# huzaifakhan04/truely-real-time-ai-generated-video-detection-framework-for-social-platforms

Measured on AMD Instinct MI355X. Metric: frames/sec (detect+embed+drift) 720p, higher is better.
Workload: dtype f32

## Files before the change

### truely-real-time-ai-generated-video-detection-framework-for-social-platforms_amd/csrc/trl_api.hip

```cpp
#include <stdarg.h>
#include <stdio.h>
#include <string.h>
#include <stdlib.h>

#include "trl_ctx.h"

static thread_local char g_err[512] = "";
int g_trl_no_fnconv = 0;
int g_trl_pnet_gate = 0;

#include <mutex>
namespace {
std::mutex g_gate_mu;
hipEvent_t g_gate_ev[64] = {};
bool g_gate_set[64] = {};
}
int trl_gate_wait(trl_ctx* c, hipStream_t s) {
    const int d = c->cfg.device;
    if (!g_trl_pnet_gate || d < 0 || d >= 64) return TRL_OK;
    std::lock_guard<std::mutex> lk(g_gate_mu);
    if (g_gate_set[d]) TRL_HIP(hipStreamWaitEvent(s, g_gate_ev[d], 0));
    return TRL_OK;
}
int trl_gate_record(trl_ctx* c, hipStream_t s) {
// ... 694 lines not shown
    TRL_HIP(hipSetDevice(c->cfg.device));
    const int capF = nb;
    Arena& A = c->arena;
    TRL_CHECK(trl_ensure(c, A, (size_t)capF * 32 + (1u << 20)));
    A.reset();
    CascadeBufs& B = c->cb;
    B = CascadeBufs();
    B.n = 1; B.H = H; B.W = W;
    B.cbox = (int32_t*)A.alloc((size_t)capF * 32);
    int32_t* total = (int32_t*)A.alloc(64);
    std::vector<int32_t> hb((size_t)nb * 8, 0);
    for (int i = 0; i < nb; i++) {
        const float* b = h_boxes + 4 * i;
        const int bx = (int)truncf(b[0]), by = (int)truncf(b[1]), bex = (int)truncf(b[2]), bey = (int)truncf(b[3]);
        const int x = bx < 1 ? 1 : bx, y = by < 1 ? 1 : by, ex = bex > W ? W : bex, ey = bey > H ? H : bey;
        hb[8 * i + 1] = y - 1; hb[8 * i + 2] = x - 1; hb[8 * i + 3] = ey - (y - 1); hb[8 * i + 4] = ex - (x - 1);
    }
    TRL_HIP(hipMemcpyAsync(B.cbox, hb.data(), hb.size() * 4, hipMemcpyHostToDevice, s));
    TRL_HIP(hipMemcpyAsync(total, &nb, 4, hipMemcpyHostToDevice, s));
    TRL_HIP(hipStreamSynchronize(s));
    c->scratch.reset();
    TRL_CHECK(trl_ensure(c, c->scratch, (size_t)nb * 700 * 1024 + (4u << 20)));
    if (net == 24) {
        float* pool1 = (float*)c->scratch.alloc((size_t)nb * 11 * 11 * 28 * 4);
        TRL_CHECK(trl_launch_rnet_front(c, d_frame, H, W, total, 0, nb, pool1, s));
        TRL_CHECK(trl_run_rnet_tail(c, pool1, nb, d_out, s, total, 0));
    } else {
        float* pool1 = (float*)c->scratch.alloc((size_t)nb * 23 * 23 * 32 * 4);
        TRL_CHECK(trl_launch_onet_front(c, d_frame, H, W, total, 0, nb, pool1, s));
        TRL_CHECK(trl_run_onet_tail(c, pool1, nb, d_out, s, total, 0));
    }
    TRL_HIP(hipStreamSynchronize(s));
    B = CascadeBufs();
    return TRL_OK;
}

int trl_debug_onet(trl_ctx* c, const float* d_crops, int n, float* d_out, void* stream) {
    if (!c || !c->have_weights || !d_crops || !d_out || n <= 0) { trl_set_error("bad argument"); return TRL_ERR_INVALID; }
    TRL_CHECK(check_idle(c));
    c->scratch.reset();
    TRL_CHECK(trl_ensure(c, c->scratch, (size_t)n * 640 * 1024 + (4u << 20)));
    return trl_run_onet(c, d_crops, n, d_out, (hipStream_t)stream);
}
int trl_debug_crop_resize(trl_ctx* c, const uint8_t* d_frames, int n, int H, int W, const int32_t* d_rect, const uint8_t* d_valid,
                          float* d_faces, void* stream) {
    if (!c || !d_frames || !d_rect || !d_valid || !d_faces || n <= 0) { trl_set_error("bad argument"); return TRL_ERR_INVALID; }
    return trl_launch_crop_resize80(d_frames, n, H, W, d_rect, d_valid, d_faces, (hipStream_t)stream);
}
int trl_debug_crop_aligned(trl_ctx* c, const uint8_t* d_frames, int n, int H, int W, const float* d_pts, const uint8_t* d_valid, int S,
                           int rgb, float* d_faces, void* stream) {
    if (!c || !d_frames || !d_pts || !d_valid || !d_faces || n <= 0 || H < 1 || W < 1 || S < 1) { trl_set_error("bad argument"); return TRL_ERR_INVALID; }
    return trl_launch_crop_aligned(d_frames, n, H, W, d_pts, d_valid, S, rgb != 0, d_faces, (hipStream_t)stream);
}
int trl_debug_nms_tiers(trl_ctx* c, int small_tier, int full_tier) {
    TRL_CHECK(check_idle(c));
    if ((small_tier && (small_tier < 16 || small_tier > 3072 || (small_tier & 3))) || (full_tier && (full_tier < 16 || full_tier > 3072 || (full_tier & 3)))) {
        trl_set_error("tiers must be multiples of 4 in [16, 3072]");
        return TRL_ERR_INVALID;
    }
    if (small_tier) c->nms_small = small_tier;
    if (full_tier) c->nms_full = full_tier;
    return TRL_OK;
}
int trl_debug_list_stats(trl_ctx* c, long long* h_out8) {
    if (!c || !h_out8) { trl_set_error("null argument"); return TRL_ERR_INVALID; }
    const int32_t* f = c->h_pinned + 4;
    unsigned long long used = 0;
    memcpy(&used, f + 8, 8);
    int mx = 0;
    for (int l = 0; l < 32; l++) if (f[16 + l] > mx) mx = f[16 + l];
    h_out8[0] = c->last_attempts; h_out8[1] = f[10]; h_out8[2] = (long long)used; h_out8[3] = (long long)c->cb.spill_cap;
    h_out8[4] = c->cb.capF; h_out8[5] = c->cb.lay.S; h_out8[6] = mx; h_out8[7] = f[6];
    return TRL_OK;
}

int trl_debug_option(trl_ctx* c, const char* key, int value) {
    if (!key) { trl_set_error("null key"); return TRL_ERR_INVALID; }
    if (!strcmp(key, "no_fnconv")) { g_trl_no_fnconv = value ? 1 : 0; return TRL_OK; }
    if (!strcmp(key, "pnet_gate")) { g_trl_pnet_gate = value ? 1 : 0; return TRL_OK; }
    TRL_CHECK(check_idle(c));
    if (!strcmp(key, "rnet_chunk") && value >= 16) { c->rnet_chunk = value; return TRL_OK; }
    if (!strcmp(key, "onet_chunk") && value >= 16) { c->onet_chunk = value; return TRL_OK; }
    if (!strcmp(key, "pnet_screen") && (value == 0 || value == 1)) { c->pnet_screen = value; return TRL_OK; }
    trl_set_error("unknown option '%s' (or value %d out of range)", key, value);
    return TRL_ERR_INVALID;
}

int trl_debug_pnet_screen_bound(trl_ctx* c, float* A, float* B, int* on) {
    if (!c || !A || !B || !on) { trl_set_error("null argument"); return TRL_ERR_INVALID; }
    *A = c->pnet_scrA; *B = c->pnet_scrB; *on = c->pnet_screen_ok && c->pnet_screen;
    return TRL_OK;
}

int trl_debug_batch_capacity(trl_ctx* c, float t2_per_frame, float t3_per_frame, int* last_attempts) {
    if (!c) { trl_set_error("null context"); return TRL_ERR_INVALID; }
    if (t2_per_frame > 0.f) c->t2_per_frame = t2_per_frame;
    if (t3_per_frame > 0.f) c->t3_per_frame = t3_per_frame;
    if (last_attempts) *last_attempts = c->last_attempts;
    return TRL_OK;
}

int trl_debug_stage_totals(trl_ctx* c, int32_t* h_out2) {
    if (!c || !h_out2) { trl_set_error("null argument"); return TRL_ERR_INVALID; }
    h_out2[0] = c->h_pinned[4 + 4]; h_out2[1] = c->h_pinned[4 + 5];
    return TRL_OK;
}

int trl_debug_pnet_run(trl_ctx* c, int run) {
    if (!c || run < 0 || run > 64) { trl_set_error("bad argument"); return TRL_ERR_INVALID; }
    c->pnet_run = run;
    return TRL_OK;
}

int trl_debug_pnet_span(trl_ctx* c, int reset, double* ms_sum, int32_t* launches) {
    if (!c || !ms_sum || !launches) { trl_set_error("null argument"); return TRL_ERR_INVALID; }
    *ms_sum = 0.0; *launches = 0;
    if (!c->pnet_clk) return TRL_OK;
    TRL_CHECK(check_idle(c));
    TRL_HIP(hipSetDevice(c->cfg.device));
    TRL_HIP(hipDeviceSynchronize());
    unsigned long long t[2] = {0, 0};
    int khz = 0;
    TRL_HIP(hipMemcpy(t, c->pnet_clk + 36, sizeof t, hipMemcpyDeviceToHost));
    TRL_HIP(hipDeviceGetAttribute(&khz, hipDeviceAttributeWallClockRate, c->cfg.device));
    if (khz > 0) *ms_sum = (double)t[0] / (double)khz;
    *launches = (int32_t)t[1];
    if (reset) TRL_HIP(hipMemset(c->pnet_clk + 36, 0, 16));
    return TRL_OK;
}

int trl_debug_pnet_kernel_ms(trl_ctx* c, float* ms) {
    if (!c || !ms) { trl_set_error("null argument"); return TRL_ERR_INVALID; }
    *ms = c->pnet_kernel_ms;
    return TRL_OK;
}

int trl_debug_timings(trl_ctx* c, float* out4) {
    if (!c || !out4) return TRL_ERR_INVALID;
    out4[0] = c->last_ms[0]; out4[1] = c->last_ms[1]; out4[2] = c->last_ms[2]; out4[3] = c->last_ms[3];
    return TRL_OK;
}

}
```

### truely-real-time-ai-generated-video-detection-framework-for-social-platforms_amd/csrc/trl_cascade.hip

```cpp
#include "trl_ctx.h"
#include <stdlib.h>
#include <string.h>


namespace {

__device__ __forceinline__ uint32_t f2ord(float f) {
    uint32_t u = __float_as_uint(f);
    return (u & 0x80000000u) ? ~u : (u | 0x80000000u);
}

__device__ void block_bitonic(uint64_t* key, uint32_t* id, int P) {
    for (int k = 2; k <= P; k <<= 1) {
        for (int j = k >> 1; j > 0; j >>= 1) {
            for (int t = threadIdx.x; t < P; t += blockDim.x) {
                const int u = t ^ j;
                if (u > t) {
                    const bool up = ((t & k) == 0);
                    const uint64_t a = key[t], b = key[u];
                    if ((a > b) == up) {
                        key[t] = b; key[u] = a;
                        const uint32_t ia = id[t]; id[t] = id[u]; id[u] = ia;
                    }
                }
// ... 1022 lines not shown
    size_t spill = c->spill_hint;
    {
        size_t per_frame = 0;
        for (int l = 0; l < L; l++) if (G.capl[l] > lds_full) per_frame += spill_need(G.capl[l], W, H);
        if (capF > lds_full) per_frame += 3 * spill_need(capF, W, H);
        size_t up_front = per_frame * (size_t)n;
        if (up_front > (8ull << 30)) up_front = 8ull << 30;
        if (up_front > spill) spill = up_front;
    }
    Arena& A = c->arena;
    Arena& X = c->scratch;
    if (resume) {
        A.off = B.arena_mark;
        TRL_HIP(hipMemsetAsync(B.flags + FLG_T3, 0, 4, s));
        TRL_HIP(hipMemsetAsync(B.flags + FLG_T3N, 0, 4, s));
        if (resume == 2) { TRL_HIP(hipMemsetAsync(B.flags + FLG_T2, 0, 4, s)); TRL_HIP(hipMemsetAsync(B.flags + FLG_T2N, 0, 4, s)); }
    }
    const size_t need = (size_t)n * ((size_t)G.S * (sizeof(Cand) + 4) + (size_t)L * 8) + (size_t)n * capF * (5 * 3 + 10 + 8) * 4 +
                        (size_t)n * 1024 + spill + (1u << 20);
    if (!resume) {
    TRL_CHECK(trl_ensure(c, A, need));
    A.reset();
    B.lvl_cnt = (int32_t*)A.alloc((size_t)n * L * 4);
    B.lvl_keep_cnt = (int32_t*)A.alloc((size_t)n * L * 4);
    B.lvl_rec = (Cand*)A.alloc((size_t)n * G.S * sizeof(Cand));
    B.lvl_keep_idx = (int32_t*)A.alloc((size_t)n * G.S * 4);
    B.n1 = (int32_t*)A.alloc((size_t)n * 4); B.n2 = (int32_t*)A.alloc((size_t)n * 4); B.n3 = (int32_t*)A.alloc((size_t)n * 4);
    B.s1_box = (float*)A.alloc((size_t)n * capF * 20); B.s2_box = (float*)A.alloc((size_t)n * capF * 20);
    B.s3_box = (float*)A.alloc((size_t)n * capF * 20); B.s3_pts = (float*)A.alloc((size_t)n * capF * 40);
    B.off2 = (int32_t*)A.alloc((size_t)(n + 1) * 4); B.off3 = (int32_t*)A.alloc((size_t)(n + 1) * 4);
    B.cbox = (int32_t*)A.alloc((size_t)n * capF * 32);
    B.flags = (int32_t*)A.alloc(TRL_NFLAGS * 4);
    B.spill = spill ? (char*)A.alloc(spill) : nullptr;
    B.spill_cap = B.spill ? spill : 0;
    if (!B.flags || (spill && !B.spill)) { trl_set_error("cascade workspace allocation failed"); return TRL_ERR_STATE; }
    B.arena_mark = A.off;
    TRL_HIP(hipMemsetAsync(B.flags, 0, TRL_NFLAGS * 4, s));
    }
    const Spill sp{B.spill, (unsigned long long)B.spill_cap, B.flags};
    if (L == 0) {
        TRL_HIP(hipMemsetAsync(B.n1, 0, (size_t)n * 4, s));
        TRL_HIP(hipMemsetAsync(B.n2, 0, (size_t)n * 4, s));
        TRL_HIP(hipMemsetAsync(B.n3, 0, (size_t)n * 4, s));
        TRL_HIP(hipMemsetAsync(B.off2, 0, (size_t)(n + 1) * 4, s));
        TRL_HIP(hipMemsetAsync(B.off3, 0, (size_t)(n + 1) * 4, s));
        if (c->scratch_after_cascade) TRL_CHECK(trl_ensure(c, X, c->scratch_after_cascade));
        return TRL_OK;
    }
    if (!resume) TRL_HIP(hipMemsetAsync(B.lvl_cnt, 0, (size_t)n * L * 4, s));

    if (!resume) c->pnet_ev_used = 0;
    X.reset();
    int chunk[32];
    const bool fused = c->cfg.pnet_mode == 0 && L <= 16;
    if (!fused) {
        size_t mx = 0;
        for (int l = 0; l < L; l++) {
            const LevelGeom& g = c->lv[l];
            const size_t per = trl_pnet_generic_bytes(1, g.h, g.w) + (size_t)g.h * g.w * 12 + (size_t)g.oh * g.ow * 24 + 4096;
            int ch = (int)((size_t)(2048ull << 20) / per);
            if (ch < 1) ch = 1;
            if (ch > n) ch = n;
            chunk[l] = ch;
            if (per * ch > mx) mx = per * ch;
        }
        TRL_CHECK(trl_ensure(c, X, mx + (4u << 20)));
    }
    auto next_ev = [&](std::pair<hipEvent_t, hipEvent_t>*& out) -> int {
        if ((int)c->pnet_ev.size() <= c->pnet_ev_used) {
            hipEvent_t e0, e1;
            TRL_HIP(hipEventCreate(&e0)); TRL_HIP(hipEventCreate(&e1));
            c->pnet_ev.push_back({e0, e1});
        }
        out = &c->pnet_ev[c->pnet_ev_used++];
        return TRL_OK;
    };
    {
        long long c2 = (long long)(c->t2_per_frame * n) + 64, c3 = (long long)(c->t3_per_frame * n) + 64;
        const long long lim = (long long)n * capF;
        c->cap_t2 = (int)(c2 < lim ? c2 : lim);
        c->cap_t3 = (int)(c3 < lim ? c3 : lim);
        const int TRL_CH2 = c->rnet_chunk, TRL_CH3 = c->onet_chunk;
        const int ch2 = c->cap_t2 < TRL_CH2 ? c->cap_t2 : TRL_CH2, ch3 = c->cap_t3 < TRL_CH3 ? c->cap_t3 : TRL_CH3;
        size_t need_x = (size_t)c->cap_t2 * 24 + (size_t)ch2 * (40 * 1024) + (1u << 20);
        const size_t need3 = (size_t)c->cap_t3 * 64 + (size_t)ch3 * (240 * 1024) + (1u << 20);
        if (need3 > need_x) need_x = need3;
        if (fused) { const size_t p = trl_pnet_fused_bytes(c, n, H, W) + (1u << 20); if (p > need_x) need_x = p; }
        if (c->scratch_after_cascade > need_x) need_x = c->scratch_after_cascade;
        TRL_CHECK(trl_ensure(c, X, need_x));
    }
    if (resume) {
    } else if (fused) {
        std::pair<hipEvent_t, hipEvent_t>*pa, *pb;
        c->pnet_ev.reserve(64);
        TRL_CHECK(next_ev(pa)); TRL_CHECK(next_ev(pb));
        hipEvent_t ev[4] = {pa->first, pa->second, pb->first, pb->second};
        TRL_CHECK(trl_pnet_fused_all(c, d_frames, n, H, W, ev, s));
    } else {
        for (int l = 0; l < L; l++) {
            const LevelGeom& g = c->lv[l];
            if (g.oh < 1 || g.ow < 1) continue;
            std::pair<hipEvent_t, hipEvent_t>* pe;
            TRL_CHECK(next_ev(pe));
            TRL_HIP(hipEventRecord(pe->first, s));
            for (int f0 = 0; f0 < n; f0 += chunk[l]) {
                const int nf = (n - f0 < chunk[l]) ? n - f0 : chunk[l];
                X.reset();
                float* lvl = (float*)X.alloc((size_t)nf * g.h * g.w * 12);
                float* heads = (float*)X.alloc((size_t)nf * g.oh * g.ow * 24);
                if (!lvl || !heads) { trl_set_error("pnet generic workspace"); return TRL_ERR_STATE; }
                TRL_CHECK(trl_launch_area_level(d_frames + (size_t)f0 * H * W * 3, nf, H, W, g.h, g.w, lvl, s));
                TRL_CHECK(trl_run_pnet_generic(c, lvl, nf, g.h, g.w, heads, s));
                const size_t total = (size_t)nf * g.oh * g.ow;
                size_t blocks = (total + 255) / 256;
                if (blocks > 16384) blocks = 16384;
                k_pnet_collect<<<(unsigned)blocks, 256, 0, s>>>(heads, nf, f0, g.oh, g.ow, (float)g.scale, c->cfg.thr0, L, l, G.capl[l],
                                                                 G.rec0[l], G.S, B.lvl_cnt, B.lvl_rec, B.flags);
                TRL_LAUNCH_CHECK();
            }
            TRL_HIP(hipEventRecord(pe->second, s));
        }
    }
    int max_capl = 4;
    for (int l = 0; l < L; l++) if (G.capl[l] > max_capl) max_capl = G.capl[l];
    const int full_l = max_capl < lds_full ? max_capl : lds_full, full_f = capF < lds_full ? capF : lds_full;
    const int th_l = max_capl > lds_full ? 1024 : 256, th_f = capF > lds_full ? 1024 : 256;
    const size_t sm_l = Smem::bytes(full_l, th_l), sm_f = Smem::bytes(full_f, th_f);
    TRL_CHECK(set_dyn_smem(k_nms_level, sm_l));
    TRL_CHECK(set_dyn_smem(k_nms_frame, sm_f));
    TRL_CHECK(set_dyn_smem(k_stage2_post, sm_f));
    TRL_CHECK(set_dyn_smem(k_stage3_post, sm_f));
    if (!resume) {
        const int small_cap = full_l < lds_small ? full_l : lds_small;
        const size_t sm_s = Smem::bytes(small_cap);
        k_nms_level<<<n * L, 256, sm_s, s>>>(G, small_cap, 0, small_cap == max_capl ? 1 : 0, W, H, B.lvl_cnt, B.lvl_rec, B.lvl_keep_cnt, B.lvl_keep_idx, B.flags, sp);
        TRL_LAUNCH_CHECK();
        if (small_cap < max_capl) {
            k_nms_level<<<n * L, th_l, sm_l, s>>>(G, full_l, small_cap + 1, 1, W, H, B.lvl_cnt, B.lvl_rec, B.lvl_keep_cnt, B.lvl_keep_idx, B.flags, sp);
            TRL_LAUNCH_CHECK();
        }
    }
    if (!resume) {
        k_nms_frame<<<n, th_f, sm_f, s>>>(G, full_f, capF, W, H, B.lvl_rec, B.lvl_keep_cnt, B.lvl_keep_idx, B.n1, B.s1_box, B.flags, sp);
        TRL_LAUNCH_CHECK();
    }

    const int cap2 = c->cap_t2, cap3 = c->cap_t3;
    if (resume < 3) {
    k_scan_counts<<<1, 256, 0, s>>>(B.n1, n, B.off2, cap2, B.flags, 0);
    TRL_LAUNCH_CHECK();
    k_build_map<<<n, 64, 0, s>>>(B.n1, B.off2, B.s1_box, capF, W, H, B.cbox);
    TRL_LAUNCH_CHECK();
    X.reset();
    float* out6 = (float*)X.alloc((size_t)cap2 * 24);
    {
        const int CH = c->rnet_chunk;
        const size_t mk = X.off;
        for (int t0 = 0; t0 < cap2; t0 += CH) {
            const int nc = (cap2 - t0 < CH) ? cap2 - t0 : CH;
            X.off = mk;
            float* pool1 = (float*)X.alloc((size_t)nc * 11 * 11 * 28 * 4);
            if (!pool1 || !out6) { trl_set_error("rnet workspace"); return TRL_ERR_STATE; }
            TRL_CHECK(trl_launch_rnet_front(c, d_frames, H, W, B.off2 + n, t0, nc, pool1, s));
            TRL_CHECK(trl_run_rnet_tail(c, pool1, nc, out6 + (size_t)t0 * 6, s, B.off2 + n, t0));
        }
    }
    k_stage2_post<<<n, th_f, sm_f, s>>>(full_f, capF, cap2, W, H, c->cfg.thr1, B.n1, B.s1_box, B.off2, out6, B.n2, B.s2_box, sp);
// ... 85 lines not shown
```

### truely-real-time-ai-generated-video-detection-framework-for-social-platforms_amd/csrc/trl_ctx.h

```cpp
#pragma once
#include "trl_common.h"

struct Cand {
    float x1, y1, x2, y2, score;
    float r0, r1, r2, r3;
    int cell;
};

struct LevelGeom {
    double scale;
    int h, w;
    int oh, ow;
};

struct LvLayout {
    int L = 0, S = 0;
    int capl[32] = {0}, rec0[32] = {0};
};
struct CascadeBufs {
    int n = 0, L = 0, H = 0, W = 0;
    LvLayout lay;
    int capF = 0;
    int32_t* lvl_cnt = nullptr;
    Cand* lvl_rec = nullptr;
    int32_t* lvl_keep_cnt = nullptr;
    int32_t* lvl_keep_idx = nullptr;
    int32_t* n1 = nullptr; float* s1_box = nullptr;
    int32_t* n2 = nullptr; float* s2_box = nullptr;
    int32_t* n3 = nullptr; float* s3_box = nullptr;
    float* s3_pts = nullptr;
    int32_t* off2 = nullptr; int32_t* off3 = nullptr;
    int32_t* cbox = nullptr;
    int32_t* flags = nullptr;
    size_t arena_mark = 0;
    char* spill = nullptr;
    size_t spill_cap = 0;
};
enum { TRL_NFLAGS = 64 };

struct trl_ctx {
    trl_config cfg;
    bool have_weights = false;
    char* wdev = nullptr;
    size_t wbytes = 0;
    std::unordered_map<std::string, DevW> W;
    std::unordered_map<std::string, DevV> V;
    Arena arena;
    Arena scratch;
    Arena sims_tmp;
    int32_t* h_pinned = nullptr;
    CascadeBufs cb;
    LevelGeom lv[32];
    hipEvent_t ev_call0 = nullptr, ev_call1 = nullptr;
    std::vector<std::pair<hipEvent_t, hipEvent_t>> pnet_ev;
    int pnet_ev_used = 0;
    float last_ms[4] = {0, 0, 0, 0};
    int pnet_mono1 = 0;
    int pnet_unit = 0;
    float pnet_scrA = 0.f, pnet_scrB = 0.f;
    int pnet_screen_ok = 0;
    int pnet_screen = 1;
    int pnet_run = 0;
    int32_t* pnet_cursor = nullptr;
    unsigned long long* pnet_clk = nullptr;
    bool pnet_prof = false;
    float pnet_kernel_ms = 0.f;
    int dbg_poison = -1;
    float t2_per_frame = 160.f, t3_per_frame = 48.f;
    int cap_t2 = 0, cap_t3 = 0;
    float lvl_hint[32] = {0}, frame_hint = 0.f;
    size_t spill_hint = 0;
    int rnet_chunk = 49152, onet_chunk = 16384;
    int nms_small = 512, nms_full = 2048;
    int last_attempts = 0;
    int resume_stage = 0;
    size_t scratch_after_cascade = 0;
    int rnet_front_mode = -1, onet_front_mode = -1;
    struct Pending {
        bool active = false; int attempt = 0;
        const uint8_t* frames = nullptr; int n = 0, H = 0, W = 0;
        float* box = nullptr; float* prob = nullptr; int32_t* rect = nullptr; uint8_t* valid = nullptr; float* emb = nullptr;
        float* faces_out = nullptr; void* stream = nullptr;
    } pend;
    uint32_t* pyr_tab = nullptr;
    int pyr_tab_H = 0, pyr_tab_W = 0;
    struct { int nlev = 0, own0 = 0, band_cols = 0, strip_rows = 0, n_bands = 0, n_strips = 0; } pyr_fine;
    struct { int L = 0; int32_t row[16][TRL_PYR_PLAN_COLS] = {}; } pyr_plan;
    std::vector<trl_fn_plan_row> fn_plan;
    int fn_cap_arm = -1;
    struct { void* p = nullptr; size_t cap = 0; int32_t dims[5] = {0, 0, 0, 0, 0}; } fn_cap[3];
};

struct TrlConvChoice { int family = 0, bm = 0, bn = 0, bk = 0, pad = 0, nz = 1; };
extern thread_local TrlConvChoice g_trl_conv_choice;

int trl_gate_wait(trl_ctx* c, hipStream_t s);
int trl_gate_record(trl_ctx* c, hipStream_t s);
extern int g_trl_pnet_gate;
int trl_ensure(trl_ctx* c, Arena& a, size_t bytes);
const DevW* trl_w(trl_ctx* c, const std::string& name);
const DevV* trl_v(trl_ctx* c, const std::string& name);

int trl_run_facenet(trl_ctx* c, const float* d_faces, int n, int h, int w, const uint8_t* d_valid, float* d_emb, hipStream_t s);
int trl_run_rnet(trl_ctx* c, const float* d_crops, int n, float* d_out6, hipStream_t s);
int trl_run_onet(trl_ctx* c, const float* d_crops, int n, float* d_out16, hipStream_t s);
int trl_run_rnet_tail(trl_ctx* c, const float* d_pool1, int n, float* d_out6, hipStream_t s, const int32_t* n_dev = nullptr, int n_base = 0);
int trl_run_onet_tail(trl_ctx* c, const float* d_pool1, int n, float* d_out16, hipStream_t s, const int32_t* n_dev = nullptr, int n_base = 0);
int trl_launch_rnet_front(trl_ctx* c, const uint8_t* d_frames, int H, int W, const int32_t* d_total, int t0, int nc, float* d_pool, hipStream_t s);
int trl_launch_onet_front(trl_ctx* c, const uint8_t* d_frames, int H, int W, const int32_t* d_total, int t0, int nc, float* d_pool, hipStream_t s);
int trl_run_pnet_generic(trl_ctx* c, const float* d_level, int nf, int h, int w, float* d_heads, hipStream_t s);
size_t trl_pnet_generic_bytes(int nf, int h, int w);

int trl_cascade_detect(trl_ctx* c, const uint8_t* d_frames, int n, int H, int W, hipStream_t s, int resume = 0);
int trl_cascade_finish(trl_ctx* c, const uint8_t* d_frames, int n, int H, int W, float* d_boxes, float* d_probs, float* d_points,
                       int32_t* d_counts, float* d_box0, float* d_prob0, int32_t* d_rect, uint8_t* d_valid, float* d_pts0, hipStream_t s);
int trl_cascade_check(trl_ctx* c, int n, int* retry);
int trl_launch_crop_resize80(const uint8_t* d_frames, int n, int H, int W, const int32_t* d_rect, const uint8_t* d_valid,
                             float* d_faces, hipStream_t s);
int trl_launch_crop_aligned(const uint8_t* d_frames, int n, int H, int W, const float* d_pts0, const uint8_t* d_valid, int S, bool rgb,
                            float* d_faces, hipStream_t s);
int trl_launch_crop_area_std(const uint8_t* d_frames, int n, int H, int W, const int32_t* d_rect, const uint8_t* d_valid, int S,
                             bool rgb, float* d_faces, hipStream_t s);
int trl_launch_area_level(const uint8_t* d_frames, int nf, int H, int W, int h, int w, float* d_level, hipStream_t s);
int trl_launch_heads_to_maps(const float* d_heads, int cells, float* d_prob, float* d_reg, hipStream_t s);
int trl_compute_levels(trl_ctx* c, int H, int W);
int trl_pnet_prepare(trl_ctx* c);
size_t trl_pnet_fused_bytes(trl_ctx* c, int n, int H, int W);
int trl_pnet_fused_all(trl_ctx* c, const uint8_t* d_frames, int n, int H, int W, hipEvent_t* ev, hipStream_t s);
int trl_pyramid_export(trl_ctx* c, const uint8_t* d_frame, int H, int W, int level, float* d_out, int* h, int* w, hipStream_t s);
int trl_pyramid_export_batch(trl_ctx* c, const uint8_t* d_frames, int n, int H, int W, float* d_out, long long* pyr_stride,
                             int32_t* h_levels, int max_levels, int* n_levels, hipStream_t s);
```

### truely-real-time-ai-generated-video-detection-framework-for-social-platforms_amd/csrc/trl_nets.hip

```cpp
#include "trl_ctx.h"
#include <stdlib.h>
#include <string.h>

thread_local TrlConvChoice g_trl_conv_choice;

namespace {

struct Runner {
    trl_ctx* c;
    hipStream_t s;
    int err = TRL_OK;
    const int32_t* m_dev = nullptr;
    int m_base = 0;
    std::vector<trl_fn_plan_row>* plan = nullptr;
    int nconv = 0;
    std::string layer;
    struct ConvMeta { int idx; std::string layer; Act x, y; bool has_res; Act res; };
    std::vector<ConvMeta> pending_meta;

    void launched(const ConvArgs& a, const ConvMeta& m) {
        if (!plan) return;
        trl_fn_plan_row r;
        memset(&r, 0, sizeof(r));
        const TrlConvChoice& ch = g_trl_conv_choice;
// ... 217 lines not shown
        Act cat = R.alloc(n, OH, OW, 896, x.bf);
        Act s0 = Runner::slice(cat, 0, 384), s1 = Runner::slice(cat, 384, 256), s2 = Runner::slice(cat, 640, 256);
        R.bconv(x, f + "mixed_6a.branch0", 3, 3, 2, 2, 0, 0, &s0);
        Act a = R.bconv(x, f + "mixed_6a.branch1.0", 1, 1, 1, 1, 0, 0);
        Act a2 = R.bconv(a, f + "mixed_6a.branch1.1", 3, 3, 1, 1, 1, 1);
        R.bconv(a2, f + "mixed_6a.branch1.2", 3, 3, 2, 2, 0, 0, &s1);
        R.pool(x, 3, 2, 0, &s2);
        x = cat;
    }
    if (R.err != TRL_OK) return R.err;
    if (x.h < 3 || x.w < 3) { trl_set_error("face crop %dx%d too small for InceptionResnetV1", h, w); return TRL_ERR_INVALID; }
    for (int i = 0; i < 10; i++) x = block17(R, x, f + "repeat_2." + std::to_string(i));
    {
        const int OH = (x.h - 3) / 2 + 1, OW = (x.w - 3) / 2 + 1;
        Act cat = R.alloc(n, OH, OW, 1792, x.bf);
        Act s0 = Runner::slice(cat, 0, 384), s1 = Runner::slice(cat, 384, 256), s2 = Runner::slice(cat, 640, 256),
            s3 = Runner::slice(cat, 896, 896);
        Act t = R.bconv(x, f + "mixed_7a.fused", 1, 1, 1, 1, 0, 0);
        Act t0 = Runner::slice(t, 0, 256), t1 = Runner::slice(t, 256, 256), t2 = Runner::slice(t, 512, 256);
        R.begin_group();
        R.bconv(t0, f + "mixed_7a.branch0.1", 3, 3, 2, 2, 0, 0, &s0);
        R.bconv(t1, f + "mixed_7a.branch1.1", 3, 3, 2, 2, 0, 0, &s1);
        Act a2 = R.bconv(t2, f + "mixed_7a.branch2.1", 3, 3, 1, 1, 1, 1);
        R.end_group();
        R.bconv(a2, f + "mixed_7a.branch2.2", 3, 3, 2, 2, 0, 0, &s2);
        R.pool(x, 3, 2, 0, &s3);
        x = cat;
    }
    for (int i = 0; i < 5; i++) x = block8(R, x, f + "repeat_3." + std::to_string(i), 0.20f, true);
    x = block8(R, x, f + "block8", 1.0f, false);
    if (R.err != TRL_OK) return R.err;
    Act g;
    if (!x.bf && x.h * x.w == 1 && x.coff == 0 && x.ld == x.c) {
        g = x;
    } else {
        g = R.alloc(n, 1, 1, x.c);
        if (R.err != TRL_OK) return R.err;
        if (x.bf) TRL_CHECK(trl_launch_gap_bf16(reinterpret_cast<const uint16_t*>(x.p), n, x.h * x.w, x.c, g.p, s, c->cfg.embed_precision));
        else TRL_CHECK(trl_launch_gap(x.p, n, x.h * x.w, x.c, g.p, s));
    }
    R.layer = f + "last_linear";
    Act e = R.conv(g, trl_w(c, f + "last_linear.w"), nullptr, trl_v(c, f + "last_bn.scale"), trl_v(c, f + "last_bn.shift"),
                   nullptr, 1, 1, 1, 1, 0, 0, TRL_ACT_NONE, nullptr, nullptr, 0.f);
    if (R.err != TRL_OK) return R.err;
    return trl_launch_l2norm512(e.p, d_valid, n, d_emb, s);
}

int trl_run_rnet(trl_ctx* c, const float* d_crops, int n, float* d_out6, hipStream_t s) {
    if (n <= 0) return TRL_OK;
    Runner R{c, s};
    Act x0; x0.p = const_cast<float*>(d_crops); x0.n = n; x0.h = 24; x0.w = 24; x0.c = 3; x0.ld = 3; x0.coff = 0;
    Act x = R.mconv(x0, "rnet", "conv1", "prelu1", 3);
    x = R.pool(x, 3, 2, 1);
    x = R.mconv(x, "rnet", "conv2", "prelu2", 3);
    x = R.pool(x, 3, 2, 1);
    x = R.mconv(x, "rnet", "conv3", "prelu3", 2);
    x = R.mconv(x, "rnet", "dense4", "prelu4", 3);
    Act out; out.p = d_out6; out.n = n; out.h = 1; out.w = 1; out.c = 6; out.ld = 6; out.coff = 0;
    R.conv(x, trl_w(c, "rnet.heads.w"), trl_v(c, "rnet.heads.b"), nullptr, nullptr, nullptr, 1, 1, 1, 1, 0, 0,
           TRL_ACT_NONE, &out, nullptr, 0.f);
    return R.err;
}

int trl_run_onet(trl_ctx* c, const float* d_crops, int n, float* d_out16, hipStream_t s) {
    if (n <= 0) return TRL_OK;
    Runner R{c, s};
    Act x0; x0.p = const_cast<float*>(d_crops); x0.n = n; x0.h = 48; x0.w = 48; x0.c = 3; x0.ld = 3; x0.coff = 0;
    Act x = R.mconv(x0, "onet", "conv1", "prelu1", 3);
    x = R.pool(x, 3, 2, 1);
    x = R.mconv(x, "onet", "conv2", "prelu2", 3);
    x = R.pool(x, 3, 2, 1);
    x = R.mconv(x, "onet", "conv3", "prelu3", 3);
    x = R.pool(x, 2, 2, 1);
    x = R.mconv(x, "onet", "conv4", "prelu4", 2);
    x = R.mconv(x, "onet", "dense5", "prelu5", 3);
    Act out; out.p = d_out16; out.n = n; out.h = 1; out.w = 1; out.c = 16; out.ld = 16; out.coff = 0;
    R.conv(x, trl_w(c, "onet.heads.w"), trl_v(c, "onet.heads.b"), nullptr, nullptr, nullptr, 1, 1, 1, 1, 0, 0,
           TRL_ACT_NONE, &out, nullptr, 0.f);
    return R.err;
}

int trl_run_rnet_tail(trl_ctx* c, const float* d_pool1, int n, float* d_out6, hipStream_t s, const int32_t* n_dev, int n_base) {
    if (n <= 0) return TRL_OK;
    Runner R{c, s};
    R.m_dev = n_dev; R.m_base = n_base;
    Act x; x.p = const_cast<float*>(d_pool1); x.n = n; x.h = 11; x.w = 11; x.c = 28; x.ld = 28; x.coff = 0;
    x = R.mconv(x, "rnet", "conv2", "prelu2", 3);
    x = R.pool(x, 3, 2, 1);
    x = R.mconv(x, "rnet", "conv3", "prelu3", 2);
    x = R.mconv(x, "rnet", "dense4", "prelu4", 3);
    Act out; out.p = d_out6; out.n = n; out.h = 1; out.w = 1; out.c = 6; out.ld = 6; out.coff = 0;
    R.conv(x, trl_w(c, "rnet.heads.w"), trl_v(c, "rnet.heads.b"), nullptr, nullptr, nullptr, 1, 1, 1, 1, 0, 0,
           TRL_ACT_NONE, &out, nullptr, 0.f);
    return R.err;
}
int trl_run_onet_tail(trl_ctx* c, const float* d_pool1, int n, float* d_out16, hipStream_t s, const int32_t* n_dev, int n_base) {
    if (n <= 0) return TRL_OK;
    Runner R{c, s};
    R.m_dev = n_dev; R.m_base = n_base;
    Act x; x.p = const_cast<float*>(d_pool1); x.n = n; x.h = 23; x.w = 23; x.c = 32; x.ld = 32; x.coff = 0;
    x = R.mconv(x, "onet", "conv2", "prelu2", 3);
    x = R.pool(x, 3, 2, 1);
    x = R.mconv(x, "onet", "conv3", "prelu3", 3);
    x = R.pool(x, 2, 2, 1);
    x = R.mconv(x, "onet", "conv4", "prelu4", 2);
    x = R.mconv(x, "onet", "dense5", "prelu5", 3);
    Act out; out.p = d_out16; out.n = n; out.h = 1; out.w = 1; out.c = 16; out.ld = 16; out.coff = 0;
    R.conv(x, trl_w(c, "onet.heads.w"), trl_v(c, "onet.heads.b"), nullptr, nullptr, nullptr, 1, 1, 1, 1, 0, 0,
           TRL_ACT_NONE, &out, nullptr, 0.f);
    return R.err;
}

size_t trl_pnet_generic_bytes(int nf, int h, int w) {
    const size_t c1 = (size_t)(h - 2) * (w - 2) * 10, ph = (h - 2 + 1) / 2, pw = (w - 2 + 1) / 2;
    const size_t p1 = ph * pw * 10, c2 = (ph - 2) * (pw - 2) * 16, c3 = (ph - 4) * (pw - 4) * 32;
    return (size_t)nf * (c1 + p1 + c2 + c3) * sizeof(float) + 4096;
}

int trl_run_pnet_generic(trl_ctx* c, const float* d_level, int nf, int h, int w, float* d_heads, hipStream_t s) {
    Runner R{c, s};
    Act x0; x0.p = const_cast<float*>(d_level); x0.n = nf; x0.h = h; x0.w = w; x0.c = 3; x0.ld = 3; x0.coff = 0;
    Act x = R.mconv(x0, "pnet", "conv1", "prelu1", 3);
    x = R.pool(x, 2, 2, 1);
    x = R.mconv(x, "pnet", "conv2", "prelu2", 3);
    x = R.mconv(x, "pnet", "conv3", "prelu3", 3);
    Act out; out.p = d_heads; out.n = nf; out.h = x.h; out.w = x.w; out.c = 6; out.ld = 6; out.coff = 0;
    R.conv(x, trl_w(c, "pnet.heads.w"), trl_v(c, "pnet.heads.b"), nullptr, nullptr, nullptr, 1, 1, 1, 1, 0, 0,
           TRL_ACT_NONE, &out, nullptr, 0.f);
    return R.err;
}
```

Before: 20530.

## Fuse RNet tail layers into single MFMA kernel with LDS-staged weights

```diff
diff --git a/truely-real-time-ai-generated-video-detection-framework-for-social-platforms_amd/csrc/trl_api.hip b/truely-real-time-ai-generated-video-detection-framework-for-social-platforms_amd/csrc/trl_api.hip
--- a/truely-real-time-ai-generated-video-detection-framework-for-social-platforms_amd/csrc/trl_api.hip
+++ b/truely-real-time-ai-generated-video-detection-framework-for-social-platforms_amd/csrc/trl_api.hip
@@ -800,6 +800,8 @@
     if (!strcmp(key, "rnet_chunk") && value >= 16) { c->rnet_chunk = value; return TRL_OK; }
     if (!strcmp(key, "onet_chunk") && value >= 16) { c->onet_chunk = value; return TRL_OK; }
     if (!strcmp(key, "pnet_screen") && (value == 0 || value == 1)) { c->pnet_screen = value; return TRL_OK; }
+    if (!strcmp(key, "mtcnn_tail_layered") && (value == 0 || value == 1)) { c->tail_layered = value; return TRL_OK; }
+    if (!strcmp(key, "rnet_tail_passes") && value >= 0 && value <= 5) { c->rnet_tail_passes = value; return TRL_OK; }
     trl_set_error("unknown option '%s' (or value %d out of range)", key, value);
     return TRL_ERR_INVALID;
 }
diff --git a/truely-real-time-ai-generated-video-detection-framework-for-social-platforms_amd/csrc/trl_cascade.hip b/truely-real-time-ai-generated-video-detection-framework-for-social-platforms_amd/csrc/trl_cascade.hip
--- a/truely-real-time-ai-generated-video-detection-framework-for-social-platforms_amd/csrc/trl_cascade.hip
+++ b/truely-real-time-ai-generated-video-detection-framework-for-social-platforms_amd/csrc/trl_cascade.hip
@@ -1128,7 +1128,8 @@
         c->cap_t3 = (int)(c3 < lim ? c3 : lim);
         const int TRL_CH2 = c->rnet_chunk, TRL_CH3 = c->onet_chunk;
         const int ch2 = c->cap_t2 < TRL_CH2 ? c->cap_t2 : TRL_CH2, ch3 = c->cap_t3 < TRL_CH3 ? c->cap_t3 : TRL_CH3;
-        size_t need_x = (size_t)c->cap_t2 * 24 + (size_t)ch2 * (40 * 1024) + (1u << 20);
+        const size_t per2 = c->tail_layered ? 40 * 1024 : 14 * 1024;
+        size_t need_x = (size_t)c->cap_t2 * 24 + (size_t)ch2 * per2 + (1u << 20);
         const size_t need3 = (size_t)c->cap_t3 * 64 + (size_t)ch3 * (240 * 1024) + (1u << 20);
         if (need3 > need_x) need_x = need3;
         if (fused) { const size_t p = trl_pnet_fused_bytes(c, n, H, W) + (1u << 20); if (p > need_x) need_x = p; }
diff --git a/truely-real-time-ai-generated-video-detection-framework-for-social-platforms_amd/csrc/trl_ctx.h b/truely-real-time-ai-generated-video-detection-framework-for-social-platforms_amd/csrc/trl_ctx.h
--- a/truely-real-time-ai-generated-video-detection-framework-for-social-platforms_amd/csrc/trl_ctx.h
+++ b/truely-real-time-ai-generated-video-detection-framework-for-social-platforms_amd/csrc/trl_ctx.h
@@ -60,6 +60,9 @@
     float pnet_scrA = 0.f, pnet_scrB = 0.f;
     int pnet_screen_ok = 0;
     int pnet_screen = 1;
+    int tail_layered = 0;
+    int rnet_tail_passes = 0;
+    int n_cu = 0;
     int pnet_run = 0;
     int32_t* pnet_cursor = nullptr;
     unsigned long long* pnet_clk = nullptr;
@@ -106,6 +109,12 @@
 int trl_run_onet(trl_ctx* c, const float* d_crops, int n, float* d_out16, hipStream_t s);
 int trl_run_rnet_tail(trl_ctx* c, const float* d_pool1, int n, float* d_out6, hipStream_t s, const int32_t* n_dev = nullptr, int n_base = 0);
 int trl_run_onet_tail(trl_ctx* c, const float* d_pool1, int n, float* d_out16, hipStream_t s, const int32_t* n_dev = nullptr, int n_base = 0);
+__host__ __device__ static inline int trl_rnet_tail_passes(int n, int cus) {
+    const long long per = 3LL * 4 * (cus > 0 ? cus : 1);
+    const long long p = n / per;
+    return p < 1 ? 1 : (p > 5 ? 5 : (int)p);
+}
+int trl_launch_rnet_tail(trl_ctx* c, const float* d_pool1, int n, float* d_out6, hipStream_t s, const int32_t* n_dev, int n_base);
 int trl_launch_rnet_front(trl_ctx* c, const uint8_t* d_frames, int H, int W, const int32_t* d_total, int t0, int nc, float* d_pool, hipStream_t s);
 int trl_launch_onet_front(trl_ctx* c, const uint8_t* d_frames, int H, int W, const int32_t* d_total, int t0, int nc, float* d_pool, hipStream_t s);
 int trl_run_pnet_generic(trl_ctx* c, const float* d_level, int nf, int h, int w, float* d_heads, hipStream_t s);
diff --git a/truely-real-time-ai-generated-video-detection-framework-for-social-platforms_amd/csrc/trl_nets.hip b/truely-real-time-ai-generated-video-detection-framework-for-social-platforms_amd/csrc/trl_nets.hip
--- a/truely-real-time-ai-generated-video-detection-framework-for-social-platforms_amd/csrc/trl_nets.hip
+++ b/truely-real-time-ai-generated-video-detection-framework-for-social-platforms_amd/csrc/trl_nets.hip
@@ -323,6 +323,7 @@
 
 int trl_run_rnet_tail(trl_ctx* c, const float* d_pool1, int n, float* d_out6, hipStream_t s, const int32_t* n_dev, int n_base) {
     if (n <= 0) return TRL_OK;
+    if (!c->tail_layered) return trl_launch_rnet_tail(c, d_pool1, n, d_out6, s, n_dev, n_base);
     Runner R{c, s};
     R.m_dev = n_dev; R.m_base = n_base;
     Act x; x.p = const_cast<float*>(d_pool1); x.n = n; x.h = 11; x.w = 11; x.c = 28; x.ld = 28; x.coff = 0;
diff --git a/truely-real-time-ai-generated-video-detection-framework-for-social-platforms_amd/csrc/trl_tail.hip b/truely-real-time-ai-generated-video-detection-framework-for-social-platforms_amd/csrc/trl_tail.hip
--- /dev/null
+++ b/truely-real-time-ai-generated-video-detection-framework-for-social-platforms_amd/csrc/trl_tail.hip
@@ -0,0 +1,261 @@
+#include "trl_ctx.h"
+
+typedef float f32x4r __attribute__((ext_vector_type(4)));
+
+namespace {
+
+constexpr int RT_SUB = 3;
+constexpr int RT_PASSES = 5;
+constexpr int RT_G = RT_SUB * RT_PASSES;
+constexpr int RT_X = 11 * 11 * 28;
+constexpr int RT_Y = 81 * 48;
+constexpr int RT_PPIX = 52;
+constexpr int RT_PS = 16 * RT_PPIX + 4;
+constexpr int RT_C3S = 9 * 64 + 4;
+constexpr int RT_W2 = 252 * 48;
+constexpr int RT_XY = RT_SUB * RT_Y;
+constexpr int RT_P = RT_G * RT_PS;
+constexpr size_t RT_LDS_BYTES = (size_t)(RT_W2 + RT_XY + RT_P) * sizeof(float);
+static_assert(RT_SUB * RT_X <= RT_XY && RT_G * RT_C3S <= RT_XY, "XY region");
+static_assert(4 * 16 * 128 <= RT_W2 && RT_G * 128 <= RT_P, "aliased regions");
+static_assert((RT_SUB * RT_X) % 4 == 0 && RT_X % 4 == 0, "float4 staging");
+
+struct RTailArgs {
+    const float* x;
+    const float* w2; const float* b2; const float* s2; int ld2;
+    const float* w3; const float* b3; const float* s3; int ld3;
+    const float* w4; const float* b4; const float* s4; int ld4;
+    const float* wh; const float* bh; int ldh;
+    float* out;
+    int n;
+    const int32_t* n_dev; int n_base;
+    int passes;
+    int cus;
+};
+
+__global__ __launch_bounds__(512) void k_rnet_tail(RTailArgs a) {
+    extern __shared__ __attribute__((aligned(16))) float rt_sm[];
+    float* sW = rt_sm;
+    float* sXY = rt_sm + RT_W2;
+    float* sP = sXY + RT_XY;
+
+    int live = a.n;
+    if (a.n_dev) { const int t = *a.n_dev - a.n_base; live = t < 0 ? 0 : (t > a.n ? a.n : t); }
+    const int passes = a.passes > 0 ? a.passes : trl_rnet_tail_passes(live, a.cus);
+    const int G = RT_SUB * passes;
+    const int cand0 = blockIdx.x * G;
+    if (cand0 >= live) return;
+    const int nl = live - cand0 < G ? live - cand0 : G;
+
+    const int tid = threadIdx.x, lane = tid & 63, wave = __builtin_amdgcn_readfirstlane(tid >> 6);
+    const int l15 = lane & 15, kq = lane >> 4;
+
+    for (int e = tid; e < RT_W2 / 4; e += 512) {
+        const int k = e / 12, n4 = e - k * 12;
+        *reinterpret_cast<f32x4r*>(&sW[4 * e]) = *reinterpret_cast<const f32x4r*>(a.w2 + (size_t)k * a.ld2 + 4 * n4);
+    }
+    constexpr int XV = RT_SUB * RT_X / 4, XPT = (XV + 511) / 512;
+    f32x4r xr[XPT];
+    auto load_pass = [&](int pass) __attribute__((always_inline)) {
+        const float* src = a.x + (size_t)(cand0 + pass * RT_SUB) * RT_X;
+        const int ncand = nl - pass * RT_SUB;
+#pragma unroll
+        for (int i = 0; i < XPT; i++) {
+            const int e = tid + 512 * i;
+            f32x4r v = {0.f, 0.f, 0.f, 0.f};
+            if (e < XV && e < ncand * (RT_X / 4)) v = *reinterpret_cast<const f32x4r*>(src + 4 * e);
+            xr[i] = v;
+        }
+    };
+    auto store_pass = [&]() __attribute__((always_inline)) {
+#pragma unroll
+        for (int i = 0; i < XPT; i++) {
+            const int e = tid + 512 * i;
+            if (e < XV) *reinterpret_cast<f32x4r*>(&sXY[4 * e]) = xr[i];
+        }
+    };
+
+    int abase[2];
+#pragma unroll
+    for (int t = 0; t < 2; t++) {
+        int m = (2 * wave + t) * 16 + l15;
+        m = m < RT_SUB * 81 ? m : 0;
+        const int cd = m / 81, p = m - cd * 81, oy = p / 9, ox = p - oy * 9;
+        abase[t] = cd * RT_X + (oy * 11 + ox) * 28 + kq;
+    }
+    float b2v[3];
+#pragma unroll
+    for (int tn = 0; tn < 3; tn++) b2v[tn] = a.b2[tn * 16 + l15];
+
+    load_pass(0);
+    for (int pass = 0; pass < passes; pass++) {
+        if (pass * RT_SUB >= nl) break;
+        store_pass();
+        __syncthreads();
+        if ((pass + 1) * RT_SUB < nl) load_pass(pass + 1);
+
+        f32x4r acc[2][3];
+#pragma unroll
+        for (int t = 0; t < 2; t++)
+#pragma unroll
+            for (int tn = 0; tn < 3; tn++) acc[t][tn] = f32x4r{b2v[tn], b2v[tn], b2v[tn], b2v[tn]};
+#pragma unroll
+        for (int s = 0; s < 63; s++) {
+            const int tap = s / 7, c0 = (s - tap * 7) * 4, ky = tap / 3, kx = tap - ky * 3;
+            const int off = (ky * 11 + kx) * 28 + c0;
+            float av[2], bv[3];
+#pragma unroll
+            for (int t = 0; t < 2; t++) av[t] = sXY[abase[t] + off];
+#pragma unroll
+            for (int tn = 0; tn < 3; tn++) bv[tn] = sW[(4 * s + kq) * 48 + tn * 16 + l15];
+#pragma unroll
+            for (int t = 0; t < 2; t++)
+#pragma unroll
+                for (int tn = 0; tn < 3; tn++) acc[t][tn] = __builtin_amdgcn_mfma_f32_16x16x4f32(av[t], bv[tn], acc[t][tn], 0, 0, 0);
+        }
+        __syncthreads();
+#pragma unroll
+        for (int t = 0; t < 2; t++)
+#pragma unroll
+            for (int q = 0; q < 4; q++) {
+                const int m = (2 * wave + t) * 16 + kq * 4 + q;
+                if (m < RT_SUB * 81) {
+#pragma unroll
+                    for (int tn = 0; tn < 3; tn++) sXY[m * 48 + tn * 16 + l15] = acc[t][tn][q];
+                }
+            }
+        __syncthreads();
+        for (int e = tid; e < RT_SUB * 16 * 48; e += 512) {
+            const int c = e % 48, r = e / 48, cd = r >> 4, py = (r >> 2) & 3, px = r & 3;
+            const float* y = sXY + cd * RT_Y + ((2 * py) * 9 + 2 * px) * 48 + c;
+            float mx = y[0], mn = y[0];
+#pragma unroll
+            for (int dy = 0; dy < 3; dy++)
+#pragma unroll
+                for (int dx = 0; dx < 3; dx++) {
+                    if (dy == 0 && dx == 0) continue;
+                    const float v = y[(dy * 9 + dx) * 48];
+                    mx = vmax_nc(mx, v); mn = vmin_nc(mn, v);
+                }
+            const float sl = a.s2[c];
+            sP[(pass * RT_SUB + cd) * RT_PS + (py * 4 + px) * RT_PPIX + c] = trl_prelu_pooled(mx, mn, sl, trl_prelu_sel(sl));
+        }
+        __syncthreads();
+    }
+
+    {
+        const int tn = wave & 3, tm0 = wave >> 2;
+        int pbase[5];
+#pragma unroll
+        for (int j = 0; j < 5; j++) {
+            int m = (tm0 + 2 * j) * 16 + l15;
+            m = m < RT_G * 9 ? m : RT_G * 9 - 1;
+            const int cd = m / 9, p = m - cd * 9, oy = p / 3, ox = p - oy * 3;
+            pbase[j] = cd * RT_PS + (oy * 4 + ox) * RT_PPIX + kq;
+        }
+        const int nj = tm0 == 0 ? 5 : 4;
+        const float b = a.b3[tn * 16 + l15];
+        f32x4r acc[5];
+#pragma unroll
+        for (int j = 0; j < 5; j++) acc[j] = f32x4r{b, b, b, b};
+        const float* wcol = a.w3 + (size_t)kq * a.ld3 + tn * 16 + l15;
+#pragma unroll 12
+        for (int s = 0; s < 48; s++) {
+            const int tap = s / 12, c0 = (s - tap * 12) * 4, ky = tap >> 1, kx = tap & 1;
+            const int off = (ky * 4 + kx) * RT_PPIX + c0;
+            const float bv = wcol[(size_t)(4 * s) * a.ld3];
+#pragma unroll
+            for (int j = 0; j < 4; j++) acc[j] = __builtin_amdgcn_mfma_f32_16x16x4f32(sP[pbase[j] + off], bv, acc[j], 0, 0, 0);
+            if (nj == 5) acc[4] = __builtin_amdgcn_mfma_f32_16x16x4f32(sP[pbase[4] + off], bv, acc[4], 0, 0, 0);
+        }
+        const int n = tn * 16 + l15;
+        const float sl = a.s3[n];
+#pragma unroll
+        for (int j = 0; j < 5; j++) {
+            if (j >= nj) break;
+#pragma unroll
+            for (int q = 0; q < 4; q++) {
+                const int m = (tm0 + 2 * j) * 16 + kq * 4 + q;
+                if (m >= RT_G * 9) continue;
+                const int cd = m / 9, p = m - cd * 9;
+                float v = acc[j][q];
+                v = v > 0.f ? v : sl * v;
+                sXY[cd * RT_C3S + p * 64 + n] = v;
+            }
+        }
+    }
+    __syncthreads();
+
+    {
+        const int n = wave * 16 + l15;
+        const int row = l15 < RT_G ? l15 : RT_G - 1;
+        const float* arow = sXY + row * RT_C3S + kq;
+        const float* wcol = a.w4 + (size_t)kq * a.ld4 + n;
+        f32x4r acc[4];
+        const float b = a.b4[n];
+        acc[0] = f32x4r{b, b, b, b};
+#pragma unroll
+        for (int q = 1; q < 4; q++) acc[q] = f32x4r{0.f, 0.f, 0.f, 0.f};
+#pragma unroll 6
+        for (int s = 0; s < 36; s++) {
+#pragma unroll
+            for (int q = 0; q < 4; q++) {
+                const int k0 = q * 144 + 4 * s;
+                acc[q] = __builtin_amdgcn_mfma_f32_16x16x4f32(arow[k0], wcol[(size_t)k0 * a.ld4], acc[q], 0, 0, 0);
+            }
+        }
+        float* part = sW;
+#pragma unroll
+        for (int q = 0; q < 4; q++)
+#pragma unroll
+            for (int i = 0; i < 4; i++) part[(q * 16 + kq * 4 + i) * 128 + n] = acc[q][i];
+    }
+    __syncthreads();
+    float* d4 = sP;
+    for (int e = tid; e < RT_G * 128; e += 512) {
+        const int n = e & 127;
+        float v = (sW[e] + sW[2048 + e]) + (sW[4096 + e] + sW[6144 + e]);
+        v = v > 0.f ? v : a.s4[n] * v;
+        d4[e] = v;
+    }
+    __syncthreads();
+
+    if (tid < nl * 6) {
+        const int cd = tid / 6, j = tid - cd * 6;
+        const float* x = d4 + cd * 128;
+        float v = a.bh[j];
+#pragma unroll 8
+        for (int k = 0; k < 128; k++) v = __builtin_fmaf(x[k], a.wh[(size_t)k * a.ldh + j], v);
+        a.out[(size_t)(cand0 + cd) * 6 + j] = v;
+    }
+}
+
+}
+
+int trl_launch_rnet_tail(trl_ctx* c, const float* d_pool1, int n, float* d_out6, hipStream_t s, const int32_t* n_dev, int n_base) {
+    const DevW *w2 = trl_w(c, "rnet.conv2.w"), *w3 = trl_w(c, "rnet.conv3.w"), *w4 = trl_w(c, "rnet.dense4.w"), *wh = trl_w(c, "rnet.heads.w");
+    const DevV *b2 = trl_v(c, "rnet.conv2.b"), *b3 = trl_v(c, "rnet.conv3.b"), *b4 = trl_v(c, "rnet.dense4.b"), *bh = trl_v(c, "rnet.heads.b");
+    const DevV *s2 = trl_v(c, "rnet.prelu2"), *s3 = trl_v(c, "rnet.prelu3"), *s4 = trl_v(c, "rnet.prelu4");
+    if (!w2 || !w3 || !w4 || !wh || !b2 || !b3 || !b4 || !bh || !s2 || !s3 || !s4) {
+        trl_set_error("rnet tail weights missing");
+        return TRL_ERR_WEIGHTS;
+    }
+    if (w2->K != 252 || w2->Cout != 48 || w3->K != 192 || w3->Cout != 64 || w4->K != 576 || w4->Cout != 128 || wh->K != 128 ||
+        wh->Cout != 6 || w2->ld % 4 != 0) {
+        trl_set_error("rnet tail: unexpected layer shapes");
+        return TRL_ERR_WEIGHTS;
+    }
+    TRL_HIP(hipFuncSetAttribute(reinterpret_cast<const void*>(k_rnet_tail), hipFuncAttributeMaxDynamicSharedMemorySize, (int)RT_LDS_BYTES));
+    RTailArgs a;
+    a.x = d_pool1;
+    a.w2 = w2->p; a.b2 = b2->p; a.s2 = s2->p; a.ld2 = w2->ld;
+    a.w3 = w3->p; a.b3 = b3->p; a.s3 = s3->p; a.ld3 = w3->ld;
+    a.w4 = w4->p; a.b4 = b4->p; a.s4 = s4->p; a.ld4 = w4->ld;
+    a.wh = wh->p; a.bh = bh->p; a.ldh = wh->ld;
+    a.out = d_out6; a.n = n; a.n_dev = n_dev; a.n_base = n_base;
+    if (c->n_cu <= 0) TRL_HIP(hipDeviceGetAttribute(&c->n_cu, hipDeviceAttributeMultiprocessorCount, c->cfg.device));
+    a.passes = c->rnet_tail_passes; a.cus = c->n_cu;
+    k_rnet_tail<<<(n + RT_SUB - 1) / RT_SUB, 512, RT_LDS_BYTES, s>>>(a);
+    TRL_LAUNCH_CHECK();
+    return TRL_OK;
+}
```

New measurement: 20520 (median of 6 runs). About the same (-0.0%).
